# wangchou/whisper.coreml

Hardware: AMD Instinct MI355X
Metric: xRT (audio-s/s) large-v3 beam=5 @1/2/4/8 GPU; p50 per-token decode ms (higher is better)
Workload: dtype fp16; 1 GPU; large-v3 beam=5 transcribe() of one 600 s file, 30 s clip grid, condition_on_previous_text=False, temperature=0; model=large-v3, global_batch=20, seq_len=448

## Files before the change

### whisper.coreml_amd/csrc/wh_kernels.h

```cpp
#pragma once
#include "wh_common.h"

namespace wh {

constexpr int TKP = 1536;

template <typename T>
void launch_layernorm(const float* x, T* y, const float* g, const float* b, int rows, int n, float eps,
                      const int* rows_in, hipStream_t st);
template <typename T>
void launch_resid_ln(float* x, const float* part, int nsplit, int64_t part_stride, const float* bias, T* y,
                     const float* g, const float* b, int rows, int n, float eps, hipStream_t st, int slab_half = 0);
template <typename T>
void launch_attn_enc(const T* qkv, int ld, int ns, int H, int Tlen, int nwin, int64_t wsi, const T* vt, int tkp, T* out,
                     int64_t wso, hipStream_t st);
template <typename T>
void launch_self_attn(const T* q, int ldq, const T* kc, const T* vc, const int* rw, const int* rs, const int* rp,
                      const int* anc, int anc_beams, int nbeam, int H, int ctx, T* out, int ldo, int rows,
                      hipStream_t st);
template <typename T>
int launch_self_attn_qkv(const float* part, int nsplit, int64_t part_stride, const float* bqkv, int ns, T* kc, T* vc,
                          const int* rw, const int* rs, const int* rp, const int* anc, int anc_beams, int nbeam, int H,
                          int ctx, T* out, int ldo, int rows, hipStream_t st, int slab_half = 0);
template <typename T>
void launch_reduce_store(const float* part, int nsplit, int64_t part_stride, const float* bias, T* out, int ldo, int M,
                         int N, int gelu, hipStream_t st, int slab_half = 0);
struct XQPart {
  const float* part = nullptr;
  int part_half = 0;
  int64_t stride = 0;
  int z = 0;
  const float* bias = nullptr;
  int max_rows = 0;
  float* split_rec = nullptr;
  int* split_cnt = nullptr;
  int max_pairs = 0;
  const void* qx = nullptr;
  const void* qwf = nullptr;
};
inline bool xattn_fused_q(int n, int rows_per_window, int elem_size) {
  return elem_size == 2 && n == 1280 && rows_per_window >= 1 && rows_per_window <= 8;
}
void launch_wq_frag(const void* w, void* f, int n, hipStream_t st);
constexpr int XREC = 16 * 64 + 32;
constexpr int XS_NSP = 24;
constexpr int XS_QP = 4;
int xattn_seg_grid(int npair, int nsp, int smax);
inline bool cross_attn_q_slabs(int z) { return z == 4 || z == 8 || z == 10; }
template <typename T>
void launch_cross_attn(const T* q, int ldq, const T* ck, const T* cv, int Tk, int H, int nsplit, int nwin,
                       const int* win_row0, const int* win_nrows, const int* win_slot, int64_t win_stride, float* po,
                       float* pm, float* pl, T* out, int ldo, int rows, float* qk_out, const int* qk_map, int qk_rows,
                       hipStream_t st, XQPart xq = XQPart());
template <typename T>
void launch_embed(const T* E, const T* P, int n, const int* row_tok, int* row_pos, const int* hist,
                  const int* cur_len, int G, int hctx, int pmax, float* x, int rows, hipStream_t st);
// ... 109 lines not shown
```

### whisper.coreml_amd/csrc/wh_kernels.hip

```cpp
#include "wh_kernels.h"

#include <cstdio>
#include <type_traits>
#include <cstdlib>

namespace wh {

template <typename T>
__global__ __launch_bounds__(256) void k_layernorm(const float* __restrict__ x, T* __restrict__ y, const float* __restrict__ gamma,
                                                   const float* __restrict__ beta, int rows, int n, float eps,
                                                   const int* __restrict__ rows_in) {
  const int row = blockIdx.x * 4 + (threadIdx.x >> 6);
  const int lane = threadIdx.x & 63;
  if (row >= rows) return;
  const int src = rows_in ? rows_in[row] : row;
  const float* xr = x + (int64_t)src * n;
  constexpr int MAXV = 8;
  float4_t v[MAXV];
  const int nv = n >> 2;
#pragma unroll
  for (int i = 0; i < MAXV; ++i) {
    const int c = lane + 64 * i;
    if (c < nv) v[i] = load4f(xr + 4 * c);
  }
// ... 753 lines not shown
  for (int e = 0; e < 8; ++e) o[e] = 0.f;
  for (int p0 = kg; p0 < pos; p0 += 64) {
    Frag<T> f[8];
    float pw[8];
#pragma unroll
    for (int u = 0; u < 8; ++u) {
      const int pc = min(p0 + 8 * u, plast);
      frag_load_buf(f[u], rv, baseB + slot_of[pc] + pc * ROWB + dc * TB);
      pw[u] = p0 + 8 * u < pos ? sc[pc] : 0.f;
    }
    __builtin_amdgcn_sched_barrier(0);
#pragma unroll
    for (int u = 0; u < 8; ++u)
#pragma unroll
      for (int e = 0; e < 8; ++e) o[e] += pw[u] * to_f32(f[u].v[e]);
  }
#pragma unroll
  for (int e = 0; e < 8; ++e) {
    o[e] = xor8_sum(o[e]);
    o[e] = xor16_sum(o[e]);
    o[e] = xor32_sum(o[e]);
  }
  if (kg == 0) {
    const float inv = 1.f / sum;
#pragma unroll
    for (int e = 0; e < 8; ++e) o[e] = (o[e] + e_cur * vs[dc + e]) * inv;
    T* op = out + (int64_t)row * ldo + h * 64 + dc;
    store4(op, o[0], o[1], o[2], o[3]);
    store4(op + 4, o[4], o[5], o[6], o[7]);
  }
  CT_END(CT_SELF_ATTN);
}

int self_attn_kco_min() {
  static const int v = [] {
    const char* e = tune_env("WHISPER_HIP_SA_KCO_MIN");
    return e ? atoi(e) : 64;
  }();
  return v;
}
template <typename T>
int launch_self_attn_qkv(const float* part, int nsplit, int64_t part_stride, const float* bqkv, int ns, T* kc, T* vc,
                          const int* rw, const int* rs, const int* rp, const int* anc, int anc_beams, int nbeam, int H,
                          int ctx, T* out, int ldo, int rows, hipStream_t st, int slab_half) {
  if (rows <= 0) return 0;
  if (anc_beams < 1 || rows % anc_beams || nsplit > 16) return -1;
  if (slab_half) {
    if constexpr (sizeof(T) == 2) {
      k_self_attn_qkv<T, half_t><<<rows * H, 64, 0, st>>>(reinterpret_cast<const half_t*>(part), nsplit, part_stride,
                                                         bqkv, ns, kc, vc, rw, rs, rp, anc, anc_beams, nbeam, H, ctx,
                                                         out, ldo, self_attn_kco_min()), wh_launched("k_self_attn_qkv");
      return 0;
    }
    return -1;
  }
  k_self_attn_qkv<T><<<rows * H, 64, 0, st>>>(part, nsplit, part_stride, bqkv, ns, kc, vc, rw, rs, rp, anc, anc_beams,
                                             nbeam, H, ctx, out, ldo, self_attn_kco_min()), wh_launched("k_self_attn_qkv");
  return 0;
}

template <typename T, int ACT, typename S = float>
__global__ __launch_bounds__(256) void k_reduce_store(const S* __restrict__ part, int nsplit, int64_t part_stride,
                                                      const float* __restrict__ bias, T* __restrict__ out, int ldo, int M,
                                                      int N) {
  const int i = (int)(blockIdx.x * 256 + threadIdx.x) * 4;
  CT_MARK(CT_REDUCE, 0);
  if (i >= M * N) return;
  const int m = (int)((unsigned)i / (unsigned)N), n = i - m * N;
  typedef typename std::conditional<sizeof(S) == 2, half4_t, float4_t>::type R4;
  R4 pp[16];
#pragma unroll
  for (int z = 0; z < 16; ++z)
    if (z < nsplit) pp[z] = *reinterpret_cast<const R4*>(part + z * part_stride + i);
  float4_t v = bias ? load4f(bias + n) : (float4_t){0.f, 0.f, 0.f, 0.f};
#pragma unroll
  for (int z = 0; z < 16; ++z)
    if (z < nsplit) v += (float4_t){(float)pp[z][0], (float)pp[z][1], (float)pp[z][2], (float)pp[z][3]};
  if (ACT) {
#pragma unroll
// ... 903 lines not shown
  const int64_t total = (int64_t)n_mels * count_per_row;
  for (int64_t i = (int64_t)blockIdx.x * blockDim.x + threadIdx.x; i < total; i += (int64_t)gridDim.x * blockDim.x) {
    const int m = (int)(i / count_per_row);
    const int64_t f = i - (int64_t)m * count_per_row;
    float* p = mel + (int64_t)m * ld + f;
    *p = (fmaxf(*p, floor_v) + 4.0f) * 0.25f;
  }
}

void launch_mel(const float* audio, int64_t n_real, int64_t n_padded, int64_t frame0, int64_t count,
                const float* filters, int n_mels, float* mel, int64_t ld, unsigned* gmax, hipStream_t st) {
  const int64_t nb = (count + MEL_FB - 1) / MEL_FB;
  if (nb > 0)
    k_mel_frames<<<(unsigned)nb, 256, 0, st>>>(audio, n_real, n_padded, frame0 + count, frame0, filters, n_mels, mel, ld, gmax), wh_launched("k_mel_frames");
}
void launch_mel_norm(float* mel, int64_t count, int64_t ld, int n_mels, const unsigned* gmax, const float* ovr,
                     hipStream_t st) {
  k_mel_norm<<<1024, 256, 0, st>>>(mel, count, ld, n_mels, gmax, ovr), wh_launched("k_mel_norm");
}
int mel_blocks(int64_t nframes) { return (int)((nframes + MEL_FB - 1) / MEL_FB); }
void launch_mel_seg(const float* audio, const MelFile* files, int n_files, int64_t n_blocks, const float* filters,
                    int n_mels, float* mel, int64_t ld, unsigned* gmax, hipStream_t st) {
  if (n_blocks <= 0) return;
  k_mel_frames_seg<<<(unsigned)n_blocks, 256, 0, st>>>(audio, files, n_files, filters, n_mels, mel, ld, gmax), wh_launched("k_mel_frames_seg");
  k_mel_norm_seg<<<(unsigned)n_blocks, 256, 0, st>>>(mel, ld, n_mels, files, n_files, gmax), wh_launched("k_mel_norm_seg");
}

#define INST(T)                                                                                                     \
  template void launch_layernorm<T>(const float*, T*, const float*, const float*, int, int, float, const int*,     \
                                    hipStream_t);                                                                   \
  template void launch_resid_ln<T>(float*, const float*, int, int64_t, const float*, T*, const float*, const float*, \
                                   int, int, float, hipStream_t, int);                           \
  template int launch_self_attn_qkv<T>(const float*, int, int64_t, const float*, int, T*, T*, const int*, const int*, \
                                        const int*, const int*, int, int, int, int, T*, int, int, hipStream_t, int); \
  template void launch_reduce_store<T>(const float*, int, int64_t, const float*, T*, int, int, int, int, hipStream_t, \
                                       int);                                                                        \
  template void launch_attn_enc<T>(const T*, int, int, int, int, int, int64_t, const T*, int, T*, int64_t,         \
                                   hipStream_t);                                                                    \
  template void launch_self_attn<T>(const T*, int, const T*, const T*, const int*, const int*, const int*,         \
                                    const int*, int, int, int, int, T*, int, int, hipStream_t);                          \
  template void launch_cross_attn<T>(const T*, int, const T*, const T*, int, int, int, int, const int*, const int*, \
                                     const int*, int64_t, float*, float*, float*, T*, int, int, float*,             \
                                     const int*, int, hipStream_t, XQPart);                                                 \
  template void launch_embed<T>(const T*, const T*, int, const int*, int*, const int*, const int*, int, int, int,  \
                                float*, int, hipStream_t);                                                          \
  template void launch_mel_windows<T>(const float*, int64_t, int, const int64_t*, const int*, T*, int64_t, int, int, \
                                      hipStream_t);                                                                 \
  template void launch_zero_rows<T>(T*, int64_t, int, int, int, int, hipStream_t);
INST(float)
INST(half_t)
#undef INST

}
```

### whisper.coreml_amd/csrc/wh_runtime.hip

```cpp
#include <hip/hip_runtime.h>

#include <algorithm>
#include <chrono>
#include <cmath>
#include <cstdio>
#include <cstring>
#include <set>
#include <string>
#include <vector>

#include "whisper_hip.h"
#include "wh_align.h"
#include "wh_audio.h"
#include "wh_gemm.h"
#include "wh_host.h"
#include "wh_kernels.h"

using namespace wh;

static thread_local std::string g_release_error;

namespace {

constexpr int CTX = 448;
// ... 111 lines not shown
  int64_t* d_seeks;
  int* d_segs;
  std::vector<T*> kc, vc;
  int RD;
  int PRE = PRE_ROWS;
  float *x_d, *po, *pm, *pl, *logits, *logits2, *nsp, *part;
  T *xn_d, *q_d, *att_d, *hm_d;
  int *row_tok, *row_pos, *row_win, *row_slot, *win_row0, *win_nrows, *win_slot, *rows_in, *src_rows;
  int *st_row_win, *st_row_slot, *st_win_row0, *st_win_nrows, *st_win_slot;
  int* fp_anc = nullptr;
  static constexpr int P1_SLABS = 2048;
  float* p1_slab = nullptr;
  int* p1_cnt = nullptr;
  float* ekz_slab = nullptr;
  int* ekz_cnt = nullptr;
  float* xs_rec = nullptr;
  float* x2_d = nullptr;
  int* xs_cnt = nullptr;

  XQPart step_xq(int rows_per_window) const {
    XQPart xq;
    xq.max_rows = rows_per_window;
    xq.split_rec = xs_rec;
    xq.split_cnt = xs_cnt;
    xq.max_pairs = Wcap * nh;
    return xq;
  }
  int* qk_map;
  unsigned* suppress;
  BiasRec* bias_dev = nullptr;
  DecState S;
  DecOpts O;
  int cur_nwin = 0, cur_G = 1;
  hipGraph_t graph = nullptr;
  hipGraphExec_t gexec = nullptr;
  std::vector<char> graph_key;
  int* h_done = nullptr;
  hipEvent_t poll_ev[2] = {nullptr, nullptr};

  Timer tm;
  std::vector<hipEvent_t> proj_ev;
  int proj_ev_n = 0;

  int share_weights_from(wh_ctx* src_) override {
    auto* src = dynamic_cast<Ctx<T>*>(src_);
    if (!src || src->ns != ns || src->Ld != Ld || src->La != La || src->V != V || !src->finalized)
      return fail(-2, "share_weights: a finalized context of the same dims and dtype is needed");
    conv1_w = src->conv1_w; conv2_w = src->conv2_w; E = src->E; Pdec = src->Pdec; ckv_w = src->ckv_w;
    conv1_b = src->conv1_b; conv2_b = src->conv2_b; pos_enc = src->pos_enc; lnp_g = src->lnp_g; lnp_b = src->lnp_b;
    ln_g = src->ln_g; ln_b = src->ln_b; ckv_b = src->ckv_b;
    enc = src->enc;
    dec = src->dec;
    finalized = true;
    if (shares_from) --shares_from->sharers;
    shares_from = src;
    ++src->sharers;
    return 0;
  }

  Releases rel;
  ~Ctx() override {
    if (st) rel(hipStreamSynchronize(st), "hipStreamSynchronize");
    if (gexec) rel(hipGraphExecDestroy(gexec), "hipGraphExecDestroy");
    if (graph) rel(hipGraphDestroy(graph), "hipGraphDestroy");
    if (st) rel(hipStreamDestroy(st), "hipStreamDestroy");
    if (wbase) rel(hipFree(wbase), "hipFree(weights)");
    if (abase) rel(hipFree(abase), "hipFree(activations)");
    audio.release(rel);
    scratch.release(rel, "hipFree(scratch)");
    if (h_done) rel(hipHostFree(h_done), "hipHostFree(done flags)");
    for (auto& e : poll_ev)
      if (e) rel(hipEventDestroy(e), "hipEventDestroy(poll)");
    tm.release(rel);
    (void)hipGetLastError();
    if (!rel.first.empty()) g_release_error = rel.first;
  }

  int init(int device_, const wh_dims& dims, int Wcap_, int Gcap_) {
    device = device_;
    d = dims;
    ns = d.n_text_state;
    nh = d.n_text_head;
    La = d.n_audio_layer;
    Ld = d.n_text_layer;
    V = d.n_vocab;
    n_vocab = V;
    n_mels = d.n_mels;
    if (d.n_audio_state != ns || d.n_audio_head != nh) return fail(-2, "audio/text state or head mismatch unsupported");
    if (ns != nh * 64) return fail(-2, "head dim must be 64 (decoder.py:62-64)");
    if (d.n_audio_ctx != 1500 || d.n_text_ctx != CTX) return fail(-2, "n_audio_ctx must be 1500, n_text_ctx 448");
    if (ns % 128 || ns > 2048) return fail(-2, "n_state must be a multiple of 128 and <= 2048");
    if (V > 57344) return fail(-2, "n_vocab too large");
    Wcap = Wcap_;
    Gcap = Gcap_;
    if (Wcap < 1 || Gcap < 1 || Gcap > 8) return fail(-2, "bad max_windows / max_group");
    const int kb = 128 / (int)sizeof(T);
    K1p = ((3 * n_mels + kb - 1) / kb) * kb;
// ... 422 lines not shown
    GemmArgs g;
    if (skinny) {
      int ks = 0;
      TRY(partial(xn_d, ns, W, R, N, ns, &ks));
      launch_reduce_store<T>(part, ks, (int64_t)R * N, b, out, N, R, N, gelu, st, slab_h);
    } else {
      g.out = out; g.ldo = N;
      TRY(gemm(xn_d, ns, W, b, R, N, ns, gelu ? EPI_STORE_GELU : EPI_STORE, g));
    }
    return 0;
  }

  int sa_probe_ks = 1;
  int sa_probe_half = 0;
  int dec_layers(int R, const int* rw, const int* rs, const int* rp, int ancG, int nwin, const int* wr0, const int* wnr,
                 const int* wsl, float* aqk, const int* qkmap, int qkrows, bool step = false,
                 const int* anc = nullptr) {
    const int* A = anc ? anc : S.anc;
    const int n = ns;
    const bool skinny = step && R <= 128;
    GemmArgs g;
    final_x = nullptr;
    if (step && !qkmap && p1_active(R, nwin))
      return dec_layers_p1(R, rw, rs, rp, ancG, nwin, wr0, wnr, wsl, A);
    launch_layernorm<T>(x_d, xn_d, dec[0].ln1_g, dec[0].ln1_b, R, n, 1e-5f, nullptr, st);
    for (int l = 0; l < Ld; ++l) {
      auto& e = dec[l];
      if (skinny) {
        int ks = 0;
        TRY(partial(xn_d, n, e.wqkv, R, 3 * n, n, &ks, slab16_qkv()));
        sa_probe_ks = ks;
        sa_probe_half = slab_h;
        if (launch_self_attn_qkv<T>(part, ks, (int64_t)R * 3 * n, e.bqkv, n, kc[l], vc[l], rw, rs, rp, A, ancG,
                                    Gcap, nh, CTX, att_d, n, R, st, slab_h))
          return fail(-20, "self-attention rows are not a whole number of beam groups");
      } else {
        g = GemmArgs();
        g.out = q_d; g.ldo = n; g.hs_state = n; g.hs_heads = nh;
        g.row_win = rw; g.row_slot = rs; g.row_pos = rp; g.kc = kc[l]; g.vc = vc[l]; g.kv_beams = Gcap; g.kv_ctx = CTX;
        TRY(gemm(xn_d, n, e.wqkv, e.bqkv, R, 3 * n, n, EPI_QKV_DEC, g));
        launch_self_attn<T>(q_d, n, kc[l], vc[l], rw, rs, rp, A, ancG, Gcap, nh, CTX, att_d, n, R, st);
      }
      TRY(resid(att_d, n, e.wo, e.bo, R, e.lnx_g, e.lnx_b));
      XQPart xq;
      if (skinny) xq = step_xq(ancG);
      if (skinny && xq_proj_active(ancG)) {
        xq.qx = xn_d; xq.qwf = e.wqx_f; xq.bias = e.bqx;
      } else if (skinny && xq_fused) {
        int ks = 0;
        TRY(partial(xn_d, n, e.wqx, R, n, n, &ks));
        if (cross_attn_q_slabs(ks)) {
          xq.part = part; xq.part_half = slab_h; xq.stride = (int64_t)R * n; xq.z = ks; xq.bias = e.bqx;
        } else {
          launch_reduce_store<T>(part, ks, (int64_t)R * n, e.bqx, q_d, n, R, n, 0, st, slab_h);
        }
      } else {
        TRY(proj(e.wqx, e.bqx, R, n, q_d, 0, skinny));
      }
      const T* ck = ckv + (size_t)(2 * l) * Wcap * TKP * n;
      const T* cv = ckv + (size_t)(2 * l + 1) * Wcap * TKP * n;
      launch_cross_attn<T>(q_d, n, ck, cv, 1500, nh, NSPLIT, nwin, wr0, wnr, wsl, (int64_t)TKP * n, po, pm, pl, att_d,
                           n, R, aqk, qkmap ? qkmap + l * nh : nullptr, qkrows, st, xq);
      TRY(resid(att_d, n, e.wox, e.box, R, e.ln2_g, e.ln2_b));
      TRY(proj(e.w1, e.b1, R, 4 * n, hm_d, 1, skinny));
      const bool last = l + 1 == Ld;
      TRY(resid(hm_d, 4 * n, e.w2, e.b2, R, last ? ln_g : dec[l + 1].ln1_g, last ? ln_b : dec[l + 1].ln1_b));
    }
// ... 34 lines not shown
      const Q qs[5] = {{att_d, n, e.wo, e.bo, n, EPI_RESID, nullptr, nullptr, nullptr},
                       {nullptr, n, e.wqx, e.bqx, n, EPI_STORE, e.lnx_g, e.lnx_b, q_d},
                       {att_d, n, e.wox, e.box, n, EPI_RESID, nullptr, nullptr, nullptr},
                       {nullptr, n, e.w1, e.b1, 4 * n, EPI_STORE_GELU, e.ln2_g, e.ln2_b, hm_d},
                       {hm_d, 4 * n, e.w2, e.b2, n, EPI_RESID, nullptr, nullptr, nullptr}};
      for (const Q& q : qs) {
        g = GemmArgs();
        g.W = q.W; g.bias = q.b; g.M = R; g.N = q.N; g.K = q.K;
        if (q.lg) {
          g.xf32 = x_d; g.ln_g = q.lg; g.ln_b = q.lb; g.ln_eps = 1e-5f; g.out = q.out; g.ldo = q.N;
        } else {
          g.X = q.X; g.ldx = q.K; g.out_f32 = x_d; g.ldo = n;
        }
        TRY(p1(g, q.epi, q.lg != nullptr));
      }
      return 0;
    }
    struct P { const T* X; int K; const T* W; int N; } ps[6] = {
        {xn_d, n, e.wqkv, 3 * n}, {att_d, n, e.wo, n}, {xn_d, n, e.wqx, n},
        {att_d, n, e.wox, n},     {xn_d, n, e.w1, 4 * n}, {hm_d, 4 * n, e.w2, n}};
    for (auto& p : ps) {
      if (p.W == e.wqx && xq_proj_active(cur_G)) continue;
      int ks = 0;
      TRY(partial(p.X, p.K, p.W, R, p.N, p.K, &ks));
    }
    return 0;
  }

  bool p1_active(int R, int n_win) const { return n_win == 1 && p1_enabled() && proj1_supported(R, ns); }
  std::string step_kernels(int n_win, int group) const override {
    const bool p1 = p1_active(n_win * group, n_win), h = sizeof(T) == 2;
    return std::string("proj=") + (p1 ? "k_proj1" : "k_proj") + ",xattn=k_xattn_seg" +
           (!p1 && xq_proj_active(group) ? "<qproj>" : "") + ",self_attn=" +
           (p1 ? (h ? "k_self_attn<kco>" : "k_self_attn") : h ? "k_self_attn_qkv<pipe+kco>" : "k_self_attn_qkv") +
           ",tail=vocab+k_logit_part";
  }

  int dec_layers_p1(int R, const int* rw, const int* rs, const int* rp, int ancG, int nwin, const int* wr0,
                    const int* wnr, const int* wsl, const int* A) {
    const int n = ns;
    float* xc = x_d;
    float* xo = x2_d;
    const float* pend = nullptr;
    auto ln_in = [&](GemmArgs& g, const float* lg, const float* lb) {
      g.xf32 = xc; g.ln_g = lg; g.ln_b = lb; g.ln_eps = 1e-5f;
      if (pend) { g.res_slab = p1_slab; g.res_bias = pend; g.x_out = xo; }
    };
    auto ln_done = [&]() {
      if (pend) { std::swap(xc, xo); pend = nullptr; }
    };
    auto resid = [&](const T* X, int K, const T* W, const float* b, bool defer) -> int {
      GemmArgs g;
      g.X = X; g.ldx = K; g.W = W; g.bias = b; g.M = R; g.N = n; g.K = K; g.out_f32 = xc; g.ldo = n;
      g.p1_defer = defer;
      TRY(p1(g, EPI_RESID, false));
      if (defer) pend = b;
      return 0;
    };
    for (int l = 0; l < Ld; ++l) {
      auto& e = dec[l];
      GemmArgs g;
      g.W = e.wqkv; g.bias = e.bqkv; g.M = R; g.N = 3 * n; g.K = n;
      ln_in(g, e.ln1_g, e.ln1_b);
      g.out = q_d; g.ldo = n; g.hs_state = n; g.hs_heads = nh;
      g.row_win = rw; g.row_slot = rs; g.row_pos = rp; g.kc = kc[l]; g.vc = vc[l]; g.kv_beams = Gcap; g.kv_ctx = CTX;
      TRY(p1(g, EPI_QKV_DEC, true));
      ln_done();
// ... 163 lines not shown
      if (rows > PRE) return fail(-11, "prefill rows exceed buffer");
      std::vector<int> sub_toks(toks.begin() + (size_t)w0 * HCTX, toks.begin() + (size_t)(w0 + nw) * HCTX);
      std::vector<int> sub_n(nin.begin() + w0, nin.begin() + w0 + nw);
      TRY(prefill(w0, nw, sub_toks, sub_n, sot_index, true));
      w0 += nw;
    }
    if (no_speech >= 0) launch_no_speech(logits2, 2 * V, n_win, V, no_speech, nsp, st);
    std::vector<int> src(n_win);
    for (int w = 0; w < n_win; ++w) src[w] = 2 * w + 1;
    HIPCHK(hipMemcpyAsync(src_rows, src.data(), n_win * 4, hipMemcpyHostToDevice, st));
    launch_broadcast_rows(logits2, V, src_rows, logits, V, G, n_win, V, st);
    HIPCHK(hipMemcpyAsync(S.hist, hist.data(), (size_t)n_win * G * HCTX * 4, hipMemcpyHostToDevice, st));
    HIPCHK(hipMemcpyAsync(S.len, nin.data(), n_win * 4, hipMemcpyHostToDevice, st));
    HIPCHK(hipMemcpyAsync(S.sample_begin, nin.data(), n_win * 4, hipMemcpyHostToDevice, st));
    HIPCHK(hipMemsetAsync(S.step, 0, n_win * 4, st));
    HIPCHK(hipMemsetAsync(S.done, 0, n_win * 4, st));
    HIPCHK(hipMemsetAsync(S.fin_n, 0, n_win * 4, st));
    HIPCHK(hipMemsetAsync(S.sum_lp, 0, n_win * G * 4, st));
    HIPCHK(hipMemcpyAsync(S.seed, &h_seed, 8, hipMemcpyHostToDevice, st));
    std::vector<int> srw(n_win * G), srs(n_win * G), swr0(n_win), swnr(n_win, G), swsl(n_win);
    for (int w = 0; w < n_win; ++w) {
      swr0[w] = w * G;
      swsl[w] = win_slots[w];
      for (int b = 0; b < G; ++b) { srw[w * G + b] = w; srs[w * G + b] = b; }
    }
    HIPCHK(hipMemcpyAsync(st_row_win, srw.data(), srw.size() * 4, hipMemcpyHostToDevice, st));
    HIPCHK(hipMemcpyAsync(st_row_slot, srs.data(), srs.size() * 4, hipMemcpyHostToDevice, st));
    HIPCHK(hipMemcpyAsync(st_win_row0, swr0.data(), n_win * 4, hipMemcpyHostToDevice, st));
    HIPCHK(hipMemcpyAsync(st_win_nrows, swnr.data(), n_win * 4, hipMemcpyHostToDevice, st));
    HIPCHK(hipMemcpyAsync(st_win_slot, swsl.data(), n_win * 4, hipMemcpyHostToDevice, st));
    cur_nwin = n_win;
    cur_G = G;
    h_len = nin;
    HIPCHK(hipStreamSynchronize(st));
    return 0;
  }

  int decode_begin(int n_win, const wh_decode_opts* o, const int* init, const int* n_init, int max_init,
                   const int* sot_index, const int* slots) override {
    if (!finalized) return fail(-9, "weights not finalized");
    if (n_win < 1 || n_win > Wcap) return fail(-11, "n_win out of range");
    TRY(set_opts(o, n_win));
    TRY(tm.mark(0, st));
    TRY(begin_batch(n_win, o->group, init, n_init, max_init, sot_index, o->no_speech, slots));
    S.maxc = std::max(maxc, 1);
    maxc_stride = S.maxc;
    step_api = false;
    launch_select_merge(logits, V, S, O, n_win, st, merge_embed());
    rows_dirty = false;
    return tm.finish(st, stats[WH_STAT_PREFILL_MS], __func__);
  }

  bool rows_dirty = false;
  void restore_rows() {
    if (!rows_dirty || cur_nwin < 1 || step_api) return;
    launch_embed<T>(E, Pdec, ns, nullptr, row_pos, S.hist, S.len, cur_G, HCTX, CTX - 1, x_d, cur_nwin * cur_G, st);
    rows_dirty = false;
  }
  MergeEmbed merge_embed() const {
    MergeEmbed em;
    em.E = E; em.P = Pdec; em.x = x_d; em.row_pos = row_pos; em.n = ns; em.pmax = CTX - 1; em.half = sizeof(T) == 2;
    return em;
  }
  int step_body() {
    const int R = cur_nwin * cur_G;
    TRY(dec_layers(R, st_row_win, st_row_slot, row_pos, cur_G, cur_nwin, st_win_row0, st_win_nrows, st_win_slot,
                   nullptr, nullptr, 0, true));
    TRY(vocab(nullptr, R, logits));
    launch_select_merge(logits, V, S, O, cur_nwin, st, merge_embed());
    return 0;
  }

  bool step_api = false;
  int step_prefill(int n_win, int G, const int* init, const int* n_init, int max_init, const int* sot_index,
                   float* lg) override {
    TRY(tm.mark(0, st));
    TRY(begin_batch(n_win, G, init, n_init, max_init, sot_index, -1));
    step_api = true;
    if (lg) HIPCHK(hipMemcpyAsync(lg, logits2, (size_t)2 * n_win * V * 4, hipMemcpyDeviceToHost, st));
    return tm.finish(st, stats[WH_STAT_PREFILL_MS], __func__);
  }

  int step_tokens(const int* tok, const int* offsets, float* lg) override {
    if (!step_api || cur_nwin < 1) return fail(-13, "no per-step batch (call wh_prefill first)");
    const int R = cur_nwin * cur_G;
    for (int r = 0; r < R; ++r)
      if (tok[r] < 0 || tok[r] >= V) return fail(-13, "step token out of vocabulary");
    for (int w = 0; w < cur_nwin; ++w) {
      if (h_len[w] >= CTX) return fail(-13, "text context full (448 positions)");
      if (offsets && offsets[w] != h_len[w])
        return fail(-13, "text_offset " + std::to_string(offsets[w]) + " of window " + std::to_string(w) +
                             " != cached length " + std::to_string(h_len[w]));
    }
    TRY(tm.mark(0, st));
    HIPCHK(hipMemcpyAsync(rows_in, tok, R * 4, hipMemcpyHostToDevice, st));
    launch_append_tokens(S, rows_in, cur_nwin, st);
    launch_embed<T>(E, Pdec, ns, nullptr, row_pos, S.hist, S.len, cur_G, HCTX, CTX - 1, x_d, R, st);
    TRY(dec_layers(R, st_row_win, st_row_slot, row_pos, cur_G, cur_nwin, st_win_row0, st_win_nrows, st_win_slot,
                   nullptr, nullptr, 0, true));
    TRY(vocab(nullptr, R, logits));
    if (lg) HIPCHK(hipMemcpyAsync(lg, logits, (size_t)R * V * 4, hipMemcpyDeviceToHost, st));
    TRY(tm.finish(st, stats[WH_STAT_STEPS_MS], __func__));
    for (auto& l : h_len) ++l;
    stats[WH_STAT_STEPS] += 1;
    return 0;
  }

  int reorder_kv(const int* src) override {
    if (!step_api || cur_nwin < 1) return fail(-13, "no per-step batch (call wh_prefill first)");
    const int R = cur_nwin * cur_G;
    for (int r = 0; r < R; ++r)
      if (src[r] / cur_G != r / cur_G || src[r] < 0)
        return fail(-13, "source row " + std::to_string(src[r]) + " of row " + std::to_string(r) +
                             " is not a row of the same window");
    HIPCHK(hipMemcpyAsync(src_rows, src, R * 4, hipMemcpyHostToDevice, st));
    launch_reorder_rows(S, src_rows, cur_nwin, st);
    HIPCHK(hipStreamSynchronize(st));
    TRY(launch_status(__func__));
    return 0;
  }

  int ensure_graph() {
    std::vector<char> key(sizeof(DecOpts) + sizeof(DecState) + 8);
    memcpy(key.data(), &O, sizeof(DecOpts));
    memcpy(key.data() + sizeof(DecOpts), &S, sizeof(DecState));
    memcpy(key.data() + sizeof(DecOpts) + sizeof(DecState), &cur_nwin, 4);
    memcpy(key.data() + sizeof(DecOpts) + sizeof(DecState) + 4, &cur_G, 4);
    if (gexec && key == graph_key) return 0;
    if (gexec) { hipGraphExecDestroy(gexec); gexec = nullptr; }
    if (graph) { hipGraphDestroy(graph); graph = nullptr; }
    HIPCHK(hipStreamBeginCapture(st, hipStreamCaptureModeThreadLocal));
    const int rc = step_body();
    hipGraph_t g = nullptr;
    const hipError_t e = hipStreamEndCapture(st, &g);
    if (rc) { if (g) hipGraphDestroy(g); return rc; }
    if (e != hipSuccess) return fail(-12, std::string("graph capture: ") + hipGetErrorString(e));
    graph = g;
    HIPCHK(hipGraphInstantiate(&gexec, graph, nullptr, nullptr, 0));
    graph_key = key;
    return 0;
  }

  const bool xq_fused = [] {
    const char* e = tune_env("WHISPER_HIP_XQ");
    return !(e && e[0] == '0');
  }();
  static bool xq_proj_on() {
    static const bool on = [] {
      const char* e = tune_env("WHISPER_HIP_XQP");
      return !(e && e[0] == '0');
    }();
    return on;
  }
  bool xq_proj_active(int rows_per_window) const {
    return xq_proj_on() && xattn_fused_q(ns, rows_per_window, (int)sizeof(T));
  }
  bool eager() const {
    const char* e = tune_env("WHISPER_HIP_EAGER");
    return e && e[0] == '1';
  }

  int launch_step() {
    if (eager()) return step_body();
    HIPCHK(hipGraphLaunch(gexec, st));
    return 0;
  }

  int decode_steps(int max_steps, int* n_done) override {
    if (cur_nwin < 1) return fail(-13, "no decode in progress");
    if (step_api) return fail(-13, "the batch was begun with wh_prefill (per-step mode): use wh_step");
    if (!eager()) TRY(ensure_graph());
    TRY(tm.mark(0, st));
    restore_rows();
    int steps = 0, done = 0;
    static const int chunk = [] {
      const char* e = tune_env("WHISPER_HIP_POLL_CHUNK");
      const int v = e ? atoi(e) : 8;
      return v < 1 ? 1 : v;
    }();
    auto queue_chunk = [&](int b) -> int {
      const int k = std::min(chunk, max_steps - steps);
      for (int i = 0; i < k; ++i) TRY(launch_step());
      steps += k;
      HIPCHK(hipMemcpyAsync(h_done + b * Wcap, S.done, cur_nwin * 4, hipMemcpyDeviceToHost, st));
      HIPCHK(hipEventRecord(poll_ev[b], st));
      return k;
    };
    auto tc = std::chrono::steady_clock::now();
    int b = 0, kq[2] = {0, 0};
    kq[0] = queue_chunk(0);
    if (kq[0] < 0) return kq[0];
    while (true) {
      const int nb = b ^ 1;
      kq[nb] = steps < max_steps ? queue_chunk(nb) : 0;
      if (kq[nb] < 0) return kq[nb];
      HIPCHK(hipEventSynchronize(poll_ev[b]));
      const auto now = std::chrono::steady_clock::now();
// ... 322 lines not shown
      HIPCHK(hipEventRecord(tm.ev[0], st));
      for (int i = 0; i < iters * (warm ? Ld : 1); ++i)
        for (int l = 0; l < nl; ++l) {
          auto& e = dec[l];
          if (what == 2) {
            TRY(layer_projections(l, R));
            launches += 6;
          } else {
            const T* ck = ckv + (size_t)(2 * l) * Wcap * TKP * n;
            const T* cv = ckv + (size_t)(2 * l + 1) * Wcap * TKP * n;
            XQPart xq = step_xq(cur_G);
            if (!p1_active(R, cur_nwin) && xq_proj_active(cur_G)) {
              xq.qx = xn_d; xq.qwf = e.wqx_f; xq.bias = e.bqx;
            }
            launch_cross_attn<T>(q_d, n, ck, cv, 1500, nh, NSPLIT, cur_nwin, st_win_row0, st_win_nrows, st_win_slot,
                                 (int64_t)TKP * n, po, pm, pl, att_d, n, R, nullptr, nullptr, 0, st, xq);
            ++launches;
          }
        }
      HIPCHK(hipEventRecord(tm.ev[1], st));
      HIPCHK(hipStreamSynchronize(st));
      float t = 0;
      HIPCHK(hipEventElapsedTime(&t, tm.ev[0], tm.ev[1]));
      *ms = t / launches;
      return 0;
    } else if (what == 7) {
      if (cur_nwin < 1) return fail(-16, "no decode batch");
      const int per_step = 6 * Ld;
      proj_ev.resize(2 * per_step * iters);
      for (auto& ev : proj_ev) HIPCHK(hipEventCreateWithFlags(&ev, hipEventDisableSystemFence));
      double tot = 0;
      int launches = 0, rc = 0;
      proj_ev_n = 0;
      for (int i = 0; i < iters && rc == 0; ++i) rc = step_body();
      if (rc == 0 && hipStreamSynchronize(st) != hipSuccess) rc = fail(-100, "time_stage(7): sync failed");
      for (int j = 0; rc == 0 && j < proj_ev_n; ++j) {
        float t = 0;
        if (hipEventElapsedTime(&t, proj_ev[2 * j], proj_ev[2 * j + 1]) != hipSuccess)
          rc = fail(-100, "time_stage(7): hipEventElapsedTime failed");
        tot += t;
        ++launches;
      }
      for (auto& ev : proj_ev)
        if (hipEventDestroy(ev) != hipSuccess && rc == 0) rc = fail(-100, "time_stage(7): hipEventDestroy failed");
      proj_ev.clear();
      proj_ev_n = 0;
      if (rc) return rc;
      *ms = launches ? tot / launches : 0.0;
      return 0;
    } else if (what == 8 || what == 9) {
      if (cur_nwin < 1 || cur_G < 1) return fail(-16, "no decode batch");
      if (p1_active(cur_nwin * cur_G, cur_nwin)) return fail(-2, "time_stage(8/9): the single-window step has no k_self_attn_qkv");
      const int R = cur_nwin * cur_G, n = ns;
      const size_t ab = (size_t)Wcap * Gcap * CTX * sizeof(int);
      int* saved = nullptr;
      if (what == 9) {
        HIPCHK(hipMalloc((void**)&saved, ab));
        HIPCHK(hipMemcpyAsync(saved, S.anc, ab, hipMemcpyDeviceToDevice, st));
        HIPCHK(hipMemsetAsync(S.anc, 0, ab, st));
      }
      int rc = 0;
      if (hipEventRecord(tm.ev[0], st) != hipSuccess) rc = fail(-100, "time_stage(8/9): hipEventRecord failed");
      for (int i = 0; rc == 0 && i < iters; ++i)
        for (int l = 0; rc == 0 && l < Ld; ++l)
          if (launch_self_attn_qkv<T>(part, sa_probe_ks, (int64_t)R * 3 * n, dec[l].bqkv, n, kc[l], vc[l], st_row_win,
                                      st_row_slot, row_pos, S.anc, cur_G, Gcap, nh, CTX, att_d, n, R, st, sa_probe_half))
            rc = fail(-20, "time_stage(8/9): self-attention launch refused");
      if (rc == 0 && hipEventRecord(tm.ev[1], st) != hipSuccess) rc = fail(-100, "time_stage(8/9): hipEventRecord failed");
      if (saved) {
        if (hipMemcpyAsync(S.anc, saved, ab, hipMemcpyDeviceToDevice, st) != hipSuccess && rc == 0)
          rc = fail(-100, "time_stage(9): ancestry restore failed");
        if (hipStreamSynchronize(st) != hipSuccess && rc == 0) rc = fail(-100, "time_stage(9): sync failed");
        if (hipFree(saved) != hipSuccess && rc == 0) rc = fail(-100, "time_stage(9): hipFree failed");
      }
      if (rc) return rc;
      HIPCHK(hipStreamSynchronize(st));
      float t = 0;
      HIPCHK(hipEventElapsedTime(&t, tm.ev[0], tm.ev[1]));
      *ms = t / (iters * Ld);
      return 0;
    } else if (what == 4) {
      if (cur_nwin < 1) return fail(-16, "no decode batch");
      HIPCHK(hipEventRecord(tm.ev[0], st));
      for (int i = 0; i < iters; ++i) launch_logit_rows(logits, V, S, O, cur_nwin, st);
      HIPCHK(hipEventRecord(tm.ev[1], st));
    } else {
      return fail(-2, "time_stage: unknown stage");
    }
    HIPCHK(hipStreamSynchronize(st));
    float t = 0;
    HIPCHK(hipEventElapsedTime(&t, tm.ev[0], tm.ev[1]));
    *ms = t / iters;
    return 0;
  }
};

template <typename T>
int create(int device, const wh_dims& dims, int max_windows, int max_group, wh_ctx** out) {
  auto c = new Ctx<T>();
// ... 310 lines not shown
```

Baseline: 760.5 audio-s/s.

## Split long-context decoder self-attention across two waves with a second captured graph

Adds a two-wave self-attention kernel that divides the key range between waves and merges their partial softmax states in shared memory. It is used once the decode context passes 64 tokens. Two HIP graphs are now captured, a short-context one and a long-context one, and each step picks between them from host-tracked lengths. The goal is shorter per-block latency for long contexts in the decode step. The cost is a second graph capture, extra barriers and an LDS merge, and possible lower occupancy.

```diff
diff --git a/whisper.coreml_amd/csrc/wh_kernels.h b/whisper.coreml_amd/csrc/wh_kernels.h
--- a/whisper.coreml_amd/csrc/wh_kernels.h
+++ b/whisper.coreml_amd/csrc/wh_kernels.h
@@ -21,7 +21,7 @@
 template <typename T>
 int launch_self_attn_qkv(const float* part, int nsplit, int64_t part_stride, const float* bqkv, int ns, T* kc, T* vc,
                           const int* rw, const int* rs, const int* rp, const int* anc, int anc_beams, int nbeam, int H,
-                          int ctx, T* out, int ldo, int rows, hipStream_t st, int slab_half = 0);
+                          int ctx, T* out, int ldo, int rows, hipStream_t st, int slab_half = 0, int split_w = 0);
 template <typename T>
 void launch_reduce_store(const float* part, int nsplit, int64_t part_stride, const float* bias, T* out, int ldo, int M,
                          int N, int gelu, hipStream_t st, int slab_half = 0);
diff --git a/whisper.coreml_amd/csrc/wh_kernels.hip b/whisper.coreml_amd/csrc/wh_kernels.hip
--- a/whisper.coreml_amd/csrc/wh_kernels.hip
+++ b/whisper.coreml_amd/csrc/wh_kernels.hip
@@ -809,6 +809,124 @@
   CT_END(CT_SELF_ATTN);
 }
 
+template <typename T, typename S, int W, int NS>
+__global__ __launch_bounds__(64 * W) __attribute__((amdgpu_waves_per_eu(2 * W))) void k_self_attn_qkv_split(
+    const S* __restrict__ part, int nsplit, int64_t part_stride, const float* __restrict__ bqkv, int ns,
+    T* __restrict__ kc, T* __restrict__ vc, const int* __restrict__ row_pos, const int* __restrict__ anc, int anc_beams,
+    int nbeam, int H, int ctx, T* __restrict__ out, int ldo) {
+  static_assert(sizeof(T) == 2, "the key-split form serves fp16 contexts");
+  __shared__ int slot_of[512];
+  __shared__ float qs[64], vs[64], pm_o[W][64], pm_m[W], pm_l[W], cur[1];
+  const int lane = threadIdx.x & 63, wv = __builtin_amdgcn_readfirstlane((int)threadIdx.x >> 6), G = anc_beams;
+  CT_MARK(CT_SELF_ATTN, 0);
+  const int L = xcd_remap(blockIdx.x, gridDim.x), sl = L % G, wh = L / G, h = wh % H, w = wh / H, row = w * G + sl;
+  const int64_t wbase = (int64_t)w * nbeam;
+  constexpr int TB = (int)sizeof(T), ROWB = 64 * TB;
+  const int slotB = H * ctx * ROWB, baseB = ((int)wbase * H + h) * ctx * ROWB;
+  const auto rk = wt_rsrc(kc), rv = wt_rsrc(vc);
+  const int pos = row_pos[row];
+  if (wv == 0) {
+    const int* an = anc + ((int64_t)w * anc_beams + sl) * ctx;
+    int sv[8];
+#pragma unroll
+    for (int i = 0; i < 8; ++i) sv[i] = an[min(lane + 64 * i, ctx - 1)];
+    const S* pr = part + (int64_t)row * 3 * ns + h * 64 + lane;
+    float qd = bqkv[h * 64 + lane], kd = bqkv[ns + h * 64 + lane], vd = bqkv[2 * ns + h * 64 + lane];
+    for (int z0 = 0; z0 < nsplit; z0 += NS) {
+      S a0[NS], a1[NS], a2[NS];
+#pragma unroll
+      for (int z = 0; z < NS; ++z) {
+        const int64_t zo = (int64_t)min(z0 + z, nsplit - 1) * part_stride;
+        a0[z] = pr[zo];
+        a1[z] = pr[zo + ns];
+        a2[z] = pr[zo + 2 * ns];
+      }
+      asm volatile("" ::"s"(pos));
+#pragma unroll
+      for (int z = 0; z < NS; ++z) asm volatile("" ::"v"(a0[z]), "v"(a1[z]), "v"(a2[z]));
+#pragma unroll
+      for (int z = 0; z < NS; ++z)
+        if (z0 + z < nsplit) {
+          qd += (float)a0[z];
+          kd += (float)a1[z];
+          vd += (float)a2[z];
+        }
+    }
+#pragma unroll
+    for (int i = 0; i < 8; ++i)
+      if (lane + 64 * i < pos) slot_of[lane + 64 * i] = sv[i] * slotB;
+    const T qT = from_f32<T>(qd), kT = from_f32<T>(kd), vT = from_f32<T>(vd);
+    const int64_t cur_off = ((wbase + sl) * H + h) * ((int64_t)ctx * 64) + (int64_t)pos * 64;
+    kc[cur_off + lane] = kT;
+    vc[cur_off + lane] = vT;
+    qs[lane] = to_f32(qT);
+    vs[lane] = to_f32(vT);
+    const float s_cur = wave_sum(to_f32(qT) * to_f32(kT));
+    if (lane == 0) cur[0] = s_cur;
+  }
+  asm volatile("s_waitcnt lgkmcnt(0)\n\ts_barrier" ::: "memory");
+  const int plast = max(pos - 1, 0);
+  const int kg = lane >> 3, dc = (lane & 7) * 8;
+  float m = cur[0], lsum = 0.f, o[8];
+#pragma unroll
+  for (int e = 0; e < 8; ++e) o[e] = 0.f;
+  float qd8[8];
+#pragma unroll
+  for (int e = 0; e < 8; ++e) qd8[e] = qs[dc + e];
+  for (int p0 = 64 * wv; p0 < pos; p0 += 64 * W) {
+    int off[8];
+#pragma unroll
+    for (int u = 0; u < 8; ++u) {
+      const int pc = min(p0 + kg + 8 * u, plast);
+      off[u] = baseB + slot_of[pc] + pc * ROWB + dc * TB;
+    }
+    Frag<T> k[8], v[8];
+#pragma unroll
+    for (int u = 0; u < 8; ++u) frag_load_buf(k[u], rk, off[u]);
+#pragma unroll
+    for (int u = 0; u < 8; ++u) frag_load_buf(v[u], rv, off[u]);
+    kco_pass<T, 8>(qd8, k, v, p0 + kg, pos, m, lsum, o);
+  }
+#pragma unroll
+  for (int e = 0; e < 8; ++e) {
+    o[e] = xor8_sum(o[e]);
+    o[e] = xor16_sum(o[e]);
+    o[e] = xor32_sum(o[e]);
+  }
+  if (kg == 0) {
+#pragma unroll
+    for (int e = 0; e < 8; ++e) pm_o[wv][dc + e] = o[e];
+  }
+  if (lane == 0) {
+    pm_m[wv] = m;
+    pm_l[wv] = lsum;
+  }
+  asm volatile("s_waitcnt lgkmcnt(0)\n\ts_barrier" ::: "memory");
+  if (wv != 0) return;
+  if (kg == 0) {
+    float M = pm_m[0];
+#pragma unroll
+    for (int j = 1; j < W; ++j) M = fmaxf(M, pm_m[j]);
+    float Ls = 0.f;
+#pragma unroll
+    for (int e = 0; e < 8; ++e) o[e] = 0.f;
+#pragma unroll
+    for (int j = 0; j < W; ++j) {
+      const float sj = __expf(pm_m[j] - M);
+      Ls += pm_l[j] * sj;
+#pragma unroll
+      for (int e = 0; e < 8; ++e) o[e] += pm_o[j][dc + e] * sj;
+    }
+    const float e_cur = __expf(cur[0] - M), inv = 1.f / (Ls + e_cur);
+#pragma unroll
+    for (int e = 0; e < 8; ++e) o[e] = (o[e] + e_cur * vs[dc + e]) * inv;
+    T* op = out + (int64_t)row * ldo + h * 64 + dc;
+    store4(op, o[0], o[1], o[2], o[3]);
+    store4(op + 4, o[4], o[5], o[6], o[7]);
+  }
+  CT_END(CT_SELF_ATTN);
+}
+
 int self_attn_kco_min() {
   static const int v = [] {
     const char* e = tune_env("WHISPER_HIP_SA_KCO_MIN");
@@ -819,9 +937,24 @@
 template <typename T>
 int launch_self_attn_qkv(const float* part, int nsplit, int64_t part_stride, const float* bqkv, int ns, T* kc, T* vc,
                           const int* rw, const int* rs, const int* rp, const int* anc, int anc_beams, int nbeam, int H,
-                          int ctx, T* out, int ldo, int rows, hipStream_t st, int slab_half) {
+                          int ctx, T* out, int ldo, int rows, hipStream_t st, int slab_half, int split_w) {
   if (rows <= 0) return 0;
-  if (anc_beams < 1 || rows % anc_beams || nsplit > 16) return -1;
+  if (anc_beams < 1 || rows % anc_beams || nsplit > 16 || nsplit < 1) return -1;
+  if (split_w) {
+    if constexpr (sizeof(T) == 2) {
+      if (split_w != 2) return -1;
+      auto go = [&](auto sp) {
+        using SP = decltype(sp);
+        k_self_attn_qkv_split<T, SP, 2, 4><<<rows * H, 128, 0, st>>>(
+            reinterpret_cast<const SP*>(part), nsplit, part_stride, bqkv, ns, kc, vc, rp, anc, anc_beams, nbeam, H, ctx,
+            out, ldo), wh_launched("k_self_attn_qkv_split");
+      };
+      if (slab_half) go(half_t());
+      else go(float());
+      return 0;
+    }
+    return -1;
+  }
   if (slab_half) {
     if constexpr (sizeof(T) == 2) {
       k_self_attn_qkv<T, half_t><<<rows * H, 64, 0, st>>>(reinterpret_cast<const half_t*>(part), nsplit, part_stride,
@@ -1791,7 +1924,7 @@
   template void launch_resid_ln<T>(float*, const float*, int, int64_t, const float*, T*, const float*, const float*, \
                                    int, int, float, hipStream_t, int);                           \
   template int launch_self_attn_qkv<T>(const float*, int, int64_t, const float*, int, T*, T*, const int*, const int*, \
-                                        const int*, const int*, int, int, int, int, T*, int, int, hipStream_t, int); \
+                                        const int*, const int*, int, int, int, int, T*, int, int, hipStream_t, int, int); \
   template void launch_reduce_store<T>(const float*, int, int64_t, const float*, T*, int, int, int, int, hipStream_t, \
                                        int);                                                                        \
   template void launch_attn_enc<T>(const T*, int, int, int, int, int, int64_t, const T*, int, T*, int64_t,         \
diff --git a/whisper.coreml_amd/csrc/wh_runtime.hip b/whisper.coreml_amd/csrc/wh_runtime.hip
--- a/whisper.coreml_amd/csrc/wh_runtime.hip
+++ b/whisper.coreml_amd/csrc/wh_runtime.hip
@@ -167,8 +167,8 @@
   DecState S;
   DecOpts O;
   int cur_nwin = 0, cur_G = 1;
-  hipGraph_t graph = nullptr;
-  hipGraphExec_t gexec = nullptr;
+  hipGraph_t graph[2] = {nullptr, nullptr};
+  hipGraphExec_t gexec[2] = {nullptr, nullptr};
   std::vector<char> graph_key;
   int* h_done = nullptr;
   hipEvent_t poll_ev[2] = {nullptr, nullptr};
@@ -196,8 +196,10 @@
   Releases rel;
   ~Ctx() override {
     if (st) rel(hipStreamSynchronize(st), "hipStreamSynchronize");
-    if (gexec) rel(hipGraphExecDestroy(gexec), "hipGraphExecDestroy");
-    if (graph) rel(hipGraphDestroy(graph), "hipGraphDestroy");
+    for (int i = 0; i < 2; ++i) {
+      if (gexec[i]) rel(hipGraphExecDestroy(gexec[i]), "hipGraphExecDestroy");
+      if (graph[i]) rel(hipGraphDestroy(graph[i]), "hipGraphDestroy");
+    }
     if (st) rel(hipStreamDestroy(st), "hipStreamDestroy");
     if (wbase) rel(hipFree(wbase), "hipFree(weights)");
     if (abase) rel(hipFree(abase), "hipFree(activations)");
@@ -686,7 +688,7 @@
         sa_probe_ks = ks;
         sa_probe_half = slab_h;
         if (launch_self_attn_qkv<T>(part, ks, (int64_t)R * 3 * n, e.bqkv, n, kc[l], vc[l], rw, rs, rp, A, ancG,
-                                    Gcap, nh, CTX, att_d, n, R, st, slab_h))
+                                    Gcap, nh, CTX, att_d, n, R, st, slab_h, sa_long ? SA_SPLIT_W : 0))
           return fail(-20, "self-attention rows are not a whole number of beam groups");
       } else {
         g = GemmArgs();
@@ -787,7 +789,7 @@
     const bool p1 = p1_active(n_win * group, n_win), h = sizeof(T) == 2;
     return std::string("proj=") + (p1 ? "k_proj1" : "k_proj") + ",xattn=k_xattn_seg" +
            (!p1 && xq_proj_active(group) ? "<qproj>" : "") + ",self_attn=" +
-           (p1 ? (h ? "k_self_attn<kco>" : "k_self_attn") : h ? "k_self_attn_qkv<pipe+kco>" : "k_self_attn_qkv") +
+           (p1 ? (h ? "k_self_attn<kco>" : "k_self_attn") : h ? sa_label() : "k_self_attn_qkv") +
            ",tail=vocab+k_logit_part";
   }
 
@@ -1017,6 +1019,7 @@
     cur_nwin = n_win;
     cur_G = G;
     h_len = nin;
+    q_steps = 0;
     HIPCHK(hipStreamSynchronize(st));
     return 0;
   }
@@ -1047,8 +1050,9 @@
     em.E = E; em.P = Pdec; em.x = x_d; em.row_pos = row_pos; em.n = ns; em.pmax = CTX - 1; em.half = sizeof(T) == 2;
     return em;
   }
-  int step_body() {
+  int step_body(bool lng) {
     const int R = cur_nwin * cur_G;
+    sa_long = lng;
     TRY(dec_layers(R, st_row_win, st_row_slot, row_pos, cur_G, cur_nwin, st_win_row0, st_win_nrows, st_win_slot,
                    nullptr, nullptr, 0, true));
     TRY(vocab(nullptr, R, logits));
@@ -1081,6 +1085,7 @@
     HIPCHK(hipMemcpyAsync(rows_in, tok, R * 4, hipMemcpyHostToDevice, st));
     launch_append_tokens(S, rows_in, cur_nwin, st);
     launch_embed<T>(E, Pdec, ns, nullptr, row_pos, S.hist, S.len, cur_G, HCTX, CTX - 1, x_d, R, st);
+    sa_long = long_ctx_now();
     TRY(dec_layers(R, st_row_win, st_row_slot, row_pos, cur_G, cur_nwin, st_win_row0, st_win_nrows, st_win_slot,
                    nullptr, nullptr, 0, true));
     TRY(vocab(nullptr, R, logits));
@@ -1111,19 +1116,40 @@
     memcpy(key.data() + sizeof(DecOpts), &S, sizeof(DecState));
     memcpy(key.data() + sizeof(DecOpts) + sizeof(DecState), &cur_nwin, 4);
     memcpy(key.data() + sizeof(DecOpts) + sizeof(DecState) + 4, &cur_G, 4);
-    if (gexec && key == graph_key) return 0;
-    if (gexec) { hipGraphExecDestroy(gexec); gexec = nullptr; }
-    if (graph) { hipGraphDestroy(graph); graph = nullptr; }
-    HIPCHK(hipStreamBeginCapture(st, hipStreamCaptureModeThreadLocal));
-    const int rc = step_body();
-    hipGraph_t g = nullptr;
-    const hipError_t e = hipStreamEndCapture(st, &g);
-    if (rc) { if (g) hipGraphDestroy(g); return rc; }
-    if (e != hipSuccess) return fail(-12, std::string("graph capture: ") + hipGetErrorString(e));
-    graph = g;
-    HIPCHK(hipGraphInstantiate(&gexec, graph, nullptr, nullptr, 0));
+    const int ng = sa_split_possible() ? 2 : 1;
+    if (gexec[0] && key == graph_key) return 0;
+    for (int i = 0; i < 2; ++i) {
+      if (gexec[i]) { hipGraphExecDestroy(gexec[i]); gexec[i] = nullptr; }
+      if (graph[i]) { hipGraphDestroy(graph[i]); graph[i] = nullptr; }
+    }
+    for (int i = 0; i < ng; ++i) {
+      HIPCHK(hipStreamBeginCapture(st, hipStreamCaptureModeThreadLocal));
+      const int rc = step_body(i == 1);
+      hipGraph_t g = nullptr;
+      const hipError_t e = hipStreamEndCapture(st, &g);
+      if (rc) { if (g) hipGraphDestroy(g); return rc; }
+      if (e != hipSuccess) return fail(-12, std::string("graph capture: ") + hipGetErrorString(e));
+      graph[i] = g;
+      HIPCHK(hipGraphInstantiate(&gexec[i], graph[i], nullptr, nullptr, 0));
+    }
     graph_key = key;
     return 0;
+  }
+
+  static constexpr int SA_SPLIT_W = 2, SA_LONG_T = 64;
+  int q_steps = 0;
+  bool sa_long = false;
+  bool sa_split_possible() const {
+    return sizeof(T) == 2 && cur_nwin >= 1 && !p1_active(cur_nwin * cur_G, cur_nwin);
+  }
+  bool long_ctx_now() const {
+    if (!sa_split_possible()) return false;
+    int mx = 0;
+    for (int w = 0; w < cur_nwin; ++w) mx = std::max(mx, h_len[w]);
+    return std::min(mx + q_steps, CTX - 1) > SA_LONG_T;
+  }
+  static std::string sa_label() {
+    return "k_self_attn_qkv<pipe+kco+split" + std::to_string(SA_SPLIT_W) + "@" + std::to_string(SA_LONG_T) + ">";
   }
 
   const bool xq_fused = [] {
@@ -1146,8 +1172,13 @@
   }
 
   int launch_step() {
-    if (eager()) return step_body();
-    HIPCHK(hipGraphLaunch(gexec, st));
+    const bool lng = long_ctx_now();
+    if (eager()) {
+      TRY(step_body(lng));
+    } else {
+      HIPCHK(hipGraphLaunch(gexec[lng], st));
+    }
+    ++q_steps;
     return 0;
   }
 
@@ -1536,7 +1567,10 @@
       double tot = 0;
       int launches = 0, rc = 0;
       proj_ev_n = 0;
-      for (int i = 0; i < iters && rc == 0; ++i) rc = step_body();
+      for (int i = 0; i < iters && rc == 0; ++i) {
+        rc = step_body(long_ctx_now());
+        ++q_steps;
+      }
       if (rc == 0 && hipStreamSynchronize(st) != hipSuccess) rc = fail(-100, "time_stage(7): sync failed");
       for (int j = 0; rc == 0 && j < proj_ev_n; ++j) {
         float t = 0;
@@ -1568,7 +1602,8 @@
       for (int i = 0; rc == 0 && i < iters; ++i)
         for (int l = 0; rc == 0 && l < Ld; ++l)
           if (launch_self_attn_qkv<T>(part, sa_probe_ks, (int64_t)R * 3 * n, dec[l].bqkv, n, kc[l], vc[l], st_row_win,
-                                      st_row_slot, row_pos, S.anc, cur_G, Gcap, nh, CTX, att_d, n, R, st, sa_probe_half))
+                                      st_row_slot, row_pos, S.anc, cur_G, Gcap, nh, CTX, att_d, n, R, st, sa_probe_half,
+                                      long_ctx_now() ? SA_SPLIT_W : 0))
             rc = fail(-20, "time_stage(8/9): self-attention launch refused");
       if (rc == 0 && hipEventRecord(tm.ev[1], st) != hipSuccess) rc = fail(-100, "time_stage(8/9): hipEventRecord failed");
       if (saved) {
```

Result: no change. 763.8 audio-s/s (median of 6 runs) (+0.4%).
